# JuliaLinearAlgebra/ArnoldiMethod.jl

Hardware: AMD Instinct MI355X
Metric: arnoldi_iters_per_sec (higher is better)
Workload: dtype f64

## Files before the change

arnoldimethod.jl_amd/_lib.py:

```python
from __future__ import annotations

import ctypes as C
import os

_HERE = os.path.dirname(os.path.abspath(__file__))
LIB_PATH = os.path.join(_HERE, "libkschur_hip.so")

KS_OK, KS_ERR_ARGUMENT, KS_ERR_DIMENSION, KS_ERR_HIP, KS_ERR_RCCL, KS_ERR_QR, KS_ERR_INTERNAL, KS_ERR_NO_DEVICE, KS_ERR_OPERATOR, KS_ERR_COMM = range(10)
KS_F64, KS_C64 = 0, 1
KS_I32, KS_I64 = 0, 1
KS_CSR, KS_CSC = 0, 1
LAYOUTS = {-1: "none", 0: "csr", 1: "csr-vi", 2: "csr-dvi", 3: "sell", 4: "sell-vi", 5: "stencil", 6: "csr-cb"}
PLAN_FACTS = ("ptr64", "ni", "nblk", "nlong", "row_gather", "nslices", "sell_entries", "ncolblocks", "cb_rpt", "cb_ni", "nstencil",
              "nstencil_local", "stencil_mask_bytes", "ndvi", "dvi_unroll")
WHICH = {"LM": 0, "LR": 1, "SR": 2, "LI": 3, "SI": 4}


class ArgumentError(ValueError):
    """Julia's ArgumentError (src/run.jl:111-116,123-124,165-174,185; src/ArnoldiMethod.jl:62-63,87-90)."""


class DimensionMismatch(ValueError):
    """Julia's DimensionMismatch (checksquare, src/run.jl:110)."""

# ... 86 lines not shown
    "ks_workspace_fused_rotations": [vp, P(C.c_int), P(C.c_int), P(C.c_int)],
    "ks_workspace_split_rotations": [vp, P(C.c_int)],
    "ks_workspace_deflated_blocks": [vp, P(C.c_int), P(C.c_int)],
    "ks_sstep_partition": [C.c_int, C.c_int, C.c_int, C.c_int, P(C.c_int), C.c_int, P(C.c_int)],
    "ks_workspace_assert_arnoldi": [vp, i32],
    "ks_workspace_provenance": [vp, P(C.c_int)],
    "ks_workspace_check_guard": [vp, P(C.c_int)],
    "ks_workspace_destroy": [vp],
    "ks_workspace_dims": [vp, P(i64), P(C.c_int), P(C.c_int), P(i64)],
    "ks_workspace_H": [vp, P(vp), P(C.c_int)],
    "ks_workspace_Q": [vp, P(vp), P(C.c_int)],
    "ks_workspace_col_ptr": [vp, i32, P(vp)],
    "ks_workspace_set_seed": [vp, u64],
    "ks_col_upload": [vp, i32, vp],
    "ks_col_download": [vp, i32, vp],
    "ks_cols_download": [vp, i32, i32, vp, i64],
    "ks_cols_upload": [vp, i32, i32, vp, i64],
    "ks_col_fill_uniform": [vp, i32, u64],
    "ks_col_norm": [vp, i32, P(dbl)],
    "ks_col_div": [vp, i32, dbl],
    "ks_col_copy": [vp, i32, i32],
    "ks_apply": [vp, vp, i32, i32],
    "ks_debug_apply_shifted": [vp, vp, i32, i32, dbl, dbl, dbl, i32],
    "ks_gemv_t": [vp, i32, i32, vp],
    "ks_gemv_n_sub": [vp, i32, i32, vp],
    "ks_rotate": [vp, i32, i32, i32, vp, i32],
    "ks_basis_times": [vp, i32, i32, vp, i32, i32, vp, i64],
    "ks_orthogonalize": [vp, i32, P(C.c_int)],
    "ks_reinitialize": [vp, i32, vp, P(C.c_int)],
    "ks_iterate_arnoldi": [vp, vp, i32, i32, P(ks_expand_stats)],
    "ks_params_default": [i64, P(ks_params)],
    "ks_partialschur": [vp, vp, P(ks_params), vp, vp, P(ks_history)],
    "ks_restart": [vp, P(ks_params), i32, P(C.c_int), P(C.c_int), P(C.c_int), vp, vp, vp],
    "ks_expand_restart": [vp, vp, P(ks_params), i32, i32, P(C.c_int), P(C.c_int), P(C.c_int), vp, vp, vp, P(ks_expand_stats), vp],
    "ks_profile_enable": [vp, i32],
    "ks_profile_reset": [vp],
    "ks_profile_get": [vp, i32, vp, vp, vp],
    "ks_residual_norms": [vp, vp, i32, P(dbl), P(dbl)],
    "ks_arnoldi_relation": [vp, vp, i32, P(dbl), P(dbl)],
    "ks_vectors_create": [vp, i64, i32, i32, P(vp)],
    "ks_vectors_destroy": [vp],
    "ks_vectors_dims": [vp, P(i64), P(C.c_int), P(C.c_int), P(i64)],
    "ks_vectors_upload": [vp, i32, i32, vp, i64],
    "ks_vectors_download": [vp, i32, i32, vp, i64],
    "ks_vectors_col_ptr": [vp, i32, P(vp)],
    "ks_basis_times_device": [vp, i32, i32, vp, i32, i32, vp],
# ... 59 lines not shown
```

arnoldimethod.jl_amd/api.py:

```python
from __future__ import annotations

import ctypes as C
import math
from dataclasses import dataclass

import numpy as np

from . import _lib
from ._lib import ArgumentError, DimensionMismatch, check

EPS = float(np.finfo(np.float64).eps)
DEFAULT_SEED = 20240917


class Target:
    name = "LM"

    def __repr__(self):
        return f"{self.name}()"


class LM(Target):
    name = "LM"

# ... 814 lines not shown
        return self.cols(0, self.maxdim + 1)

    def fill_uniform(self, j: int, seed: int):
        check(_lib.load().ks_col_fill_uniform(self._h, j, seed))

    def norm(self, j: int) -> float:
        out = C.c_double()
        check(_lib.load().ks_col_norm(self._h, j, C.byref(out)))
        return out.value

    def div(self, j: int, s: float):
        check(_lib.load().ks_col_div(self._h, j, s))

    def copy_col(self, dst: int, src: int):
        check(_lib.load().ks_col_copy(self._h, dst, src))

    def apply(self, A: Operator, jsrc: int, jdst: int):
        _check_op(_lib.load().ks_apply(A._h, self._h, jsrc, jdst), A)

    def apply_shifted(self, A: Operator, jsrc: int, jdst: int, theta, sigma: float, cacheable: bool = False):
        theta = complex(theta)
        _check_op(_lib.load().ks_debug_apply_shifted(A._h, self._h, jsrc, jdst, theta.real, theta.imag, float(sigma), int(bool(cacheable))), A)

    def gemv_t(self, j: int, jv: int) -> np.ndarray:
        h = np.empty(j, dtype=self.dtype)
        check(_lib.load().ks_gemv_t(self._h, j, jv, h.ctypes.data))
        return h

    def gemv_n_sub(self, j: int, jv: int, h):
        h = np.ascontiguousarray(np.asarray(h, dtype=self.dtype))
        check(_lib.load().ks_gemv_n_sub(self._h, j, jv, h.ctypes.data))

    def rotate(self, c0: int, Qblock):
        Qb = np.asfortranarray(np.asarray(Qblock, dtype=self.dtype))
        c, r = Qb.shape
        check(_lib.load().ks_rotate(self._h, c0, c, r, Qb.ctypes.data, c))

    def basis_times(self, c: int, Y) -> np.ndarray:
        Y = np.asarray(Y)
        ydt = np.complex128 if (Y.dtype.kind == "c" or self.dtype.kind == "c") else np.float64
        Yf = np.asfortranarray(Y.astype(ydt))
        out = np.empty((self.n, Yf.shape[1]), dtype=ydt, order="F")
        check(_lib.load().ks_basis_times(self._h, c, Yf.shape[1], Yf.ctypes.data, Yf.shape[0], _dtype_code(ydt), out.ctypes.data, self.n))
        return out

    def basis_times_device(self, c: int, Y) -> "DeviceVectors":
# ... 415 lines not shown
```

arnoldimethod.jl_amd/csrc/ks_backend.hpp:

```cpp
#pragma once
template <class T> struct HipBackend : ks::Backend<T> {
  using D = typename DevT<T>::type;
  ks_operator* op;
  ks_workspace* ws;
  HipBackend(ks_operator* o, ks_workspace* w) : op(o), ws(w) {}

  int64_t n_global() const override { return ws->n_global; }

  void iterate_arnoldi(int from, int to, const ks::Mat<T>& H, ks::ExpandStats& stats) override {
    guarded_expand([&] { iterate_arnoldi_impl(from, to, H, stats, nullptr); });
  }

  bool iterate_arnoldi_early(int from, int to, const ks::Mat<T>& H, ks::ExpandStats& stats, const std::function<void()>& early) override {
    const char* e = std::getenv("KS_EARLY_RESTART");
    const bool on = !(e && e[0] == '0');
    bool done = false;
    guarded_expand([&] { done = iterate_arnoldi_impl(from, to, H, stats, on ? &early : nullptr); });
    return done;
  }

  template <class F> void guarded_expand(F&& f) {
    try {
      f();
    } catch (...) {
// ... 270 lines not shown
    if (!(rest > 0.0)) return 0;
    int nd = 0;
    for (int j = 0; j < nl;) {
      const int w = width[j] == 2 ? 2 : 1;
      const double mag = w == 2 ? std::max(std::abs(lam[j]), std::abs(lam[j + 1])) : std::abs(lam[j]);
      const double growth = std::pow(mag / rest, std::max(1, steps - 1));
      if (!(mag > ratio * rest) || !(growth > 1e3) || nd + w > ksd::kDeflMax) break;
      for (int q = 0; q < w; ++q) ex.push_back(lam[j + q]);
      nd += w;
      j += w;
    }
    return nd;
  }

  void spec_enqueue(const ksd::BlkShifts<D>& sh, int k_now, bool from_true) {
    if (!ws->spec_on || !ws->rot_defer_on || !ws->gate_allowed || ws->sstep_eff < 8 || !op->async_capable || ws->ctx->hc.allreduce != nullptr) return;
    if (from_true && (!ws->true_start_on || ws->maxdim + 1 > 40)) return;
    const int ne = std::min(10, ws->maxdim - k_now - (sizeof(D) == 8 ? 1 : 0));
    if (ne < 2) return;
    if (!ensure_zscratch<D>(ws)) return;
    if (from_true && !true_start_enqueue<D>(ws)) return;
    char* zs = static_cast<char*>(ws->zscratch);
    op->shift_store_cacheable = true;
    for (int i = 0; i < ne; ++i) {
      op->in_scale = 1.0;
      const void* src = i == 0 ? (from_true ? static_cast<const void*>(ws->ztrue) : ws->col(ws->maxdim)) : static_cast<const void*>(zs + (size_t)(i - 1) * ws->ld * sizeof(D));
      double tre, tim;
      if constexpr (sizeof(D) == 8) { tre = sh.theta[i]; tim = 0.0; }
      else { tre = sh.theta[i].x; tim = sh.theta[i].y; }
      op->apply_shifted(src, zs + (size_t)i * ws->ld * sizeof(D), tre, tim, sh.sigma[i], ws->ld, ws->st);
    }
    ws->spec_sh.assign(reinterpret_cast<const char*>(&sh), reinterpret_cast<const char*>(&sh) + sizeof(sh));
    ws->spec_ne = ne;
    ws->spec_true = from_true;
    ws->spec_valid = true;
  }

  void relation_probe(int from, const ks::Mat<T>& H) {
    const int c = from - 2, nc = from;
    hipStream_t s_ = ws->ctx->stream;
    D* scratch = static_cast<D*>(ws->col(from));
    op->in_scale = 1.0;
    op->apply(ws->col(c), ws->col(from), nullptr);
    if (!ws->probe_dev) {
      KS_HIP(hipMalloc(&ws->probe_dev, 16 + (size_t)(ws->maxdim + 2) * 16));
      KS_HIP(hipHostMalloc(&ws->probe_host, 16 + (size_t)(ws->maxdim + 2) * 16, hipHostMallocCoherent | hipHostMallocMapped));
    }
    double* out = static_cast<double*>(ws->probe_dev);
    D* coef_d = reinterpret_cast<D*>(static_cast<char*>(ws->probe_dev) + 16);
    D* coef_h = reinterpret_cast<D*>(static_cast<char*>(ws->probe_host) + 16);
    double fro2 = 0.0;
    for (int j = 0; j < from - 1; ++j)
// ... 381 lines not shown
```

arnoldimethod.jl_amd/csrc/ks_block.hpp:

```cpp
#pragma once



inline bool blk_shape_ok(int dtype, int k, int s) { return ks_blk_shape_ok(dtype == KS_F64 ? 0 : 1, k, s); }
inline std::vector<int> blk_partition(int dtype, int k0, int count, int smax) {
  std::vector<int> out;
  int k = k0;
  while (count > 0) {
    int s = std::min(count, smax);
    while (s > 1 && !blk_shape_ok(dtype, k, s)) --s;
    if (!blk_shape_ok(dtype, k, s)) break;
    out.push_back(s);
    k += s;
    count -= s;
  }
  return out;
}

inline std::vector<std::complex<double>> leja_shifts(const std::vector<std::complex<double>>& ritz, int s, bool real) {
  std::vector<std::complex<double>> pts;
  for (auto z : ritz) {
    if (real) z = std::complex<double>(z.real(), 0.0);
    if (!std::isfinite(z.real()) || !std::isfinite(z.imag())) continue;
    bool dup = false;
// ... 102 lines not shown
  auto* bs = static_cast<ksd::BlkScratch<D>*>(ws->bscr);
  int k = from;
  int first = 1;
  for (int s : sizes) {
    const bool fuse = first && ws->rot_fuse;
    const bool split = fuse && ws->rot_split;
    const bool chain_true = fuse && ws->chain_true;
    ws->rot_fuse = false;
    ws->rot_split = false;
    ws->chain_true = false;
    char* zs = nullptr;
    if (fuse) {
      KS_REQUIRE(ws->zscratch != nullptr, KS_ERR_INTERNAL, "fused rotation without scratch columns (the adoption allocates them)");
      zs = static_cast<char*>(ws->zscratch);
    }
    if (split) {
      rotate_device<D>(ws, 0, ws->rot_cin, ws->rot_rr, ws->rot_out0, -1);
      ws->rot_split_count++;
    }
    auto zcol = [&](int i) -> void* { return fuse ? static_cast<void*>(zs + (size_t)i * ws->ld * sizeof(D)) : ws->col(k + i); };
    op->shift_store_cacheable = s >= 10;
    const int adopted = fuse ? ws->spec_adopt : 0;
    ws->spec_adopt = 0;
    for (int i = adopted; i < s; ++i) {
      double tre, tim;
      if constexpr (sizeof(D) == 8) { tre = sh.theta[i]; tim = 0.0; }
      else { tre = sh.theta[i].x; tim = sh.theta[i].y; }
      op->in_scale = 1.0;
      const void* src = i == 0 ? (fuse ? (chain_true ? static_cast<const void*>(ws->ztrue) : ws->col(ws->maxdim)) : ws->col(k - 1)) : zcol(i - 1);
      op->apply_shifted(src, zcol(i), tre, tim, sh.sigma[i], ws->ld, ws->st);
      if (ndefl > 0) {
        ProfScope ps(cx, KSP_AXPY, nb8 * 2.0 * (ndefl + 1) + nb8);
        if (!ws->defl_part) KS_HIP(hipMalloc(&ws->defl_part, (size_t)ksd::kDeflMax * (1024 + 1) * sizeof(D)));
        const int nbd = (int)std::max<int64_t>(1, std::min<int64_t>(std::min(1024, cx->num_cu * 4), (ws->n + kBlock - 1) / kBlock));
        D* zc = static_cast<D*>(zcol(i));
        const D* U = static_cast<const D*>(ws->col(0));
        D* part = static_cast<D*>(ws->defl_part);
        ksd::k_defl_dots<D><<<nbd, kBlock, 0, s_>>>(U, ws->ld, ndefl, zc, ws->n, part);
        if (!cx->distributed()) {
          ksd::k_defl_apply<D><<<nbd, kBlock, 0, s_>>>(U, ws->ld, ndefl, zc, ws->n, part, nbd, bs->cdefl + (size_t)i * ksd::kDeflMax);
        } else {
          D* red = part + (size_t)ksd::kDeflMax * 1024;
          ksd::k_defl_reduce<D><<<1, kBlock, 0, s_>>>(part, nbd, ndefl, red);
          cx->allreduce(reinterpret_cast<double*>(red), ndefl * (int)(sizeof(D) / 8));
          ksd::k_defl_apply<D><<<nbd, kBlock, 0, s_>>>(U, ws->ld, ndefl, zc, ws->n, red, 1, bs->cdefl + (size_t)i * ksd::kDeflMax);
        }
      }
    }
    if (ndefl > 0) ws->defl_blocks++;
    const int ne = k * s + s * (s + 1) / 2;
    int nb1, nb2;
    auto fin = [&](int stage, int nbp) {
// ... 61 lines not shown
```

arnoldimethod.jl_amd/csrc/ks_hip.hip:

```cpp
#include <hip/hip_runtime.h>
#include <rccl/rccl.h>

#include <signal.h>
#include <unistd.h>

#include <algorithm>
#include <chrono>
#include <cmath>
#include <cstdio>
#include <cstdlib>
#include <cstring>
#include <memory>
#include <stdexcept>
#include <string>
#include <thread>
#include <unordered_map>
#include <vector>

#include "../../include/kschur.h"
#include "ks_driver.hpp"
#include "ks_kernels.hpp"
#include "ks_spmv_march.hpp"
#include "ks_block_kernels.hpp"
#include "ks_block_launch.hpp"
// ... 998 lines not shown
    check_col(ws, jsrc);
    check_col(ws, jdst);
    KS_REQUIRE(jsrc != jdst, KS_ERR_ARGUMENT, "source and destination columns must differ");
    KS_REQUIRE(A->n_local == ws->n && A->dtype == ws->dtype, KS_ERR_DIMENSION, "operator / workspace mismatch");
    KS_REQUIRE(ws->dtype != KS_F64 || theta_im == 0.0, KS_ERR_ARGUMENT, "a Float64 product takes a real shift");
    ws->ctx->use();
    prov_drop(ws);
    materialize(ws);
    reset_state(ws);
    A->in_scale = 1.0;
    const bool saved = A->shift_store_cacheable;
    A->shift_store_cacheable = cacheable_store != 0;
    try {
      A->apply_shifted(ws->col(jsrc), ws->col(jdst), theta_re, theta_im, sigma, ws->ld, ws->st);
      KS_HIP(hipStreamSynchronize(ws->ctx->stream));
    } catch (...) {
      A->shift_store_cacheable = saved;
      throw;
    }
    A->shift_store_cacheable = saved;
  });
}

int ks_gemv_t(ks_workspace* ws, int j, int jv, void* h_host) {
  return guarded([&] {
    check_col(ws, jv);
    KS_REQUIRE(j >= 1 && j <= ws->maxdim + 1 && h_host, KS_ERR_ARGUMENT, "bad arguments");
    ws->ctx->use();
    materialize(ws);
    reset_state(ws);
    dispatch_dtype(ws->dtype, [&](auto tag) { gemv_t<typename DevT<decltype(tag)>::type>(ws, j, jv, h_host); });
  });
}

int ks_gemv_n_sub(ks_workspace* ws, int j, int jv, const void* h_host) {
  return guarded([&] {
    check_col(ws, jv);
    KS_REQUIRE(j >= 1 && j <= ws->maxdim + 1 && h_host, KS_ERR_ARGUMENT, "bad arguments");
    KS_REQUIRE(jv >= j, KS_ERR_ARGUMENT, "the updated column must not be one of the projected-out columns");
    ws->ctx->use();
    prov_drop(ws);
    materialize(ws);
    dispatch_dtype(ws->dtype, [&](auto tag) { gemv_n_sub<typename DevT<decltype(tag)>::type>(ws, j, jv, h_host); });
  });
}

// ... 698 lines not shown
```

arnoldimethod.jl_amd/csrc/ks_operators.hpp:

```cpp
#pragma once
struct ks_operator {
  ks_ctx* ctx = nullptr;
  int64_t n_local = 0, nnz = 0;
  int dtype = KS_F64;
  bool async_capable = true;
  double bytes_per_nnz = 0.0;
  double aux_bytes = 0.0;
  int layout = -1;
  double in_scale = 1.0;
  bool shift_store_cacheable = false;
  virtual ~ks_operator() = default;
  virtual void apply(const void* x, void* y, const DevState* st) = 0;
  virtual void apply_shifted(const void* x, void* y, double theta_re, double theta_im, double sigma, int64_t ld, const DevState* st);
};

namespace {

template <class D> struct CsrOp : ks_operator {
  void* rowptr = nullptr;
  bool ptr64 = false;
  int32_t* colidx = nullptr;
  D* val = nullptr;
  void* blkptr = nullptr;
  int32_t* blkrow = nullptr;
  int nblk = 0;
  std::vector<std::unique_ptr<CsrOp<D>>> cblocks;
  std::vector<char> cb_from_ghost;
  int cb_rpt = 0, cb_ni = 0;
  int ni = 7;
  bool row_gather = false;
  int nlong = 0;
  int32_t* blkpart = nullptr;
  D* lpart = nullptr;
  int32_t* lrow = nullptr;
  int32_t* lfirst = nullptr;
  int nstencil = 0;
// ... 138 lines not shown
        case 5: go(std::integral_constant<int, 5>{}, M1{}); break;
        case 6: go(std::integral_constant<int, 6>{}, M1{}); break;
        case 7: go(std::integral_constant<int, 7>{}, M1{}); break;
        default: go(std::integral_constant<int, 8>{}, M1{}); break;
      }
    }
  }
  ksd::ShiftArg<D> shift_arg() const {
    ksd::ShiftArg<D> a;
    a.on = shift_on ? 1 : 0;
    a.theta = shift_theta;
    a.sigma = shift_sigma;
    return a;
  }
  void apply_shifted(const void* xv, void* yv, double tre, double tim, double sigma, int64_t ld, const DevState* st) override {
    const int fuse = env_int("KS_SHIFT_FUSED", 1);
    const bool fused = fuse && n_local > 0 && nlong == 0;
    if (!fused) { ks_operator::apply_shifted(xv, yv, tre, tim, sigma, ld, st); return; }
    shift_on = true;
    if constexpr (sizeof(D) == 8) shift_theta = tre; else shift_theta = D{tre, tim};
    shift_sigma = sigma;
    try { apply(xv, yv, st); } catch (...) { shift_on = false; throw; }
    shift_on = false;
  }
  void apply(const void* xv, void* yv, const DevState* st) override {
    const D* x = static_cast<const D*>(xv);
    D* y = static_cast<D*>(yv);
    hipStream_t s = ctx->stream;
    const typename Halo<D>::Begun begun = halo.begin(x, st, n_local > 0 && cblocks.empty() && ndvi == 0 && nslices == 0);
    const ksd::HaloFused& hf = begun.hf;
    const D* xg = begun.xg;
    if (n_local > 0 && !cblocks.empty()) {
      ProfScope ps(ctx, KSP_SPMV, (double)nnz * bytes_per_nnz + aux_bytes + 2.0 * sizeof(D) * n_local);
      if (cb_rpt) {
        ksd::CbArgs<D> a{};
        a.nb = (int)cblocks.size();
        for (int b = 0; b < a.nb; ++b) {
          a.rowptr[b] = static_cast<const int32_t*>(cblocks[b]->rowptr);
          a.colidx[b] = cblocks[b]->colidx;
          a.val[b] = cblocks[b]->val;
          a.xb[b] = (!cb_from_ghost.empty() && cb_from_ghost[b]) ? xg : nullptr;
        }
        const int nt = (int)((n_local + (int64_t)kBlock * cb_rpt - 1) / ((int64_t)kBlock * cb_rpt));
        auto go = [&](auto ni_tag, auto rpt_tag) {
          constexpr int NI = decltype(ni_tag)::value, RPT = decltype(rpt_tag)::value;
          if constexpr ((size_t)NI * kBlock * sizeof(D) <= (size_t)ksd::kSpmvCapBytes)
// ... 424 lines not shown
```

arnoldimethod.jl_amd/csrc/ks_spmv_march.hpp:

```cpp
#pragma once

#include <algorithm>
#include <type_traits>

#include "ks_kernels.hpp"

namespace ksd {

typedef double f64x2m __attribute__((ext_vector_type(2)));

__device__ __forceinline__ double and_mask(double p, int bm) {
  const uint64_t u = __builtin_bit_cast(uint64_t, p);
  const uint32_t lo = (uint32_t)u & (uint32_t)bm, hi = (uint32_t)(u >> 32) & (uint32_t)bm;
  return __builtin_bit_cast(double, ((uint64_t)hi << 32) | lo);
}

__device__ __forceinline__ int march_tile(int xcd, int slot, int it, int S, int ntiles, int& tend) {
  const int q = ntiles >> 3, r = ntiles & 7;
  const int t0 = xcd < r ? xcd * (q + 1) : r * (q + 1) + (xcd - r) * q;
  tend = t0 + (xcd < r ? q + 1 : q);
  return t0 + slot + it * S;
}

__device__ __forceinline__ void march_ld16(f64x2m& dst, uint32_t voff, const void* sbase) {
  asm volatile("global_load_dwordx4 %0, %1, %2" : "=v"(dst) : "v"(voff), "s"(sbase) : "memory");
}
__device__ __forceinline__ void march_ld_u16(uint32_t& dst, uint32_t voff, const void* sbase) {
  asm volatile("global_load_ushort %0, %1, %2" : "=v"(dst) : "v"(voff), "s"(sbase) : "memory");
// ... 520 lines not shown
  for (;;) {
    const bool h1 = z + 1 < zi1;
    step(z, mA, mB, first, h1);
    first = false;
    if (!h1) break;
    ++z;
    const bool h2 = z + 1 < zi1;
    step(z, mB, mA, false, h2);
    if (!h2) break;
    ++z;
  }
  asm volatile("s_waitcnt vmcnt(0)" ::: "memory");
}

__device__ __forceinline__ void march_wait_vm(int c) {
  switch (c) {
    case 0: asm volatile("s_waitcnt vmcnt(0)" ::: "memory"); break;
    case 1: asm volatile("s_waitcnt vmcnt(1)" ::: "memory"); break;
    case 2: asm volatile("s_waitcnt vmcnt(2)" ::: "memory"); break;
    case 3: asm volatile("s_waitcnt vmcnt(3)" ::: "memory"); break;
    case 4: asm volatile("s_waitcnt vmcnt(4)" ::: "memory"); break;
    case 5: asm volatile("s_waitcnt vmcnt(5)" ::: "memory"); break;
    case 6: asm volatile("s_waitcnt vmcnt(6)" ::: "memory"); break;
    default: asm volatile("s_waitcnt vmcnt(7)" ::: "memory"); break;
  }
}

template <unsigned ODDM, int TILE, int TW>
__global__ void __launch_bounds__(TW)
    k_spmv_stencil_marchg(const uint16_t* __restrict__ mask2, const StencilDict<double> d, const double* __restrict__ x,
                          double* __restrict__ y, int64_t n, int nzr, const DevState* __restrict__ st, int shifted, double theta,
                          double sigma) {
  constexpr int NSLOT = 7, KOWN = 3, KFM = 0, KFP = 6;
  constexpr unsigned NEARM = 0x3eu;
  constexpr int PPL = TILE / (2 * TW), kWinB = (TILE + 512) * 8, kPieces = (TILE + 512) / 128, kWaves = TW / 64;
  constexpr int kRounds = (kPieces + kWaves - 1) / kWaves;
  static_assert(TW == 256 || TW == 512, "four or eight waves");
  static_assert((PPL == 1 || PPL == 2) && PPL * 2 * TW == TILE, "one or two pairs per lane");
  static_assert(3 * kWinB <= 60 * 1024, "three window buffers in at most 60 KiB");
  static_assert(kRounds + 2 * PPL <= 7, "march_wait_vm counts up to 7");
  if (st && st->breakdown >= 0) return;
  __shared__ __attribute__((aligned(16))) unsigned char win[3][kWinB];
  const int64_t P = d.delta[KFP];
  const int nx = d.delta[5], ny = (int)(P / nx);
  const int nz = (int)(n / P), ntp = (int)((P + TILE - 1) / TILE);
  const int xcd = blockIdx.x & 7, slot = blockIdx.x >> 3;
  int cnt;
  const int tj0 = march_tile(xcd, 0, 0, 0, ntp, cnt);
  cnt -= tj0;
  if (cnt <= 0) return;
  const int zr = slot / cnt, tile = tj0 + slot % cnt;
  if (zr >= nzr) return;
  const int za = (int)((int64_t)zr * nz / nzr), zb = (int)((int64_t)(zr + 1) * nz / nzr);
  const int64_t off0 = (int64_t)tile * TILE;
  const int wave = __builtin_amdgcn_readfirstlane(threadIdx.x >> 6);
  const uint32_t lane_w = (threadIdx.x & 63u) * 16u;
  const uint32_t win0 = (uint32_t)(uintptr_t)&win[0][0];
  const bool plain_st = (shifted & 2) != 0;
  const int nw = (kPieces - wave + kWaves - 1) / kWaves;
  uint32_t lane_b[PPL];
  bool lane_in[PPL];
  bool wave_has[PPL];
  int mA[PPL], mB[PPL];
// ... 138 lines not shown
          }
        }
      }
      v[KFM] = prev[j];
      if (i > 0) finish(z - 1, j, v[KOWN], -1);
      double s0 = 0.0, s1 = 0.0;
#pragma unroll
      for (int k = 0; k < KFP; ++k) {
        const double p0 = mul_nc(d.val[k], v[k].x), p1 = mul_nc(d.val[k], v[k].y);
        s0 = add_(s0, and_mask(p0, k == KFM ? fm : __builtin_amdgcn_sbfe(mA[j], k, 1)));
        s1 = add_(s1, and_mask(p1, k == KFM ? fm : __builtin_amdgcn_sbfe(mB[j], k, 1)));
      }
      acc[j].x = s0;
      acc[j].y = s1;
      prev[j] = v[KOWN];
    }
    bc = bc == 2 ? 0 : bc + 1;
  }
#pragma unroll
  for (int j = 0; j < PPL; ++j) finish(zi1 - 1, j, top[j], zi1 < nz ? -1 : 0);
  asm volatile("s_waitcnt vmcnt(0)" ::: "memory");
}

}
```

arnoldimethod.jl_amd/csrc/ks_stencil_geom.hpp:

```cpp
#pragma once

#include <cstddef>
#include <cstdint>

struct StencilGeom {
  bool box = false;
  int64_t nx = 0, ny = 0, nz = 0;
};

inline uint8_t stencil_box_mask(int64_t x, int64_t y, int64_t z, int64_t nx, int64_t ny, int64_t nz) {
  return (uint8_t)((z > 0 ? 0x01u : 0u) | (y > 0 ? 0x02u : 0u) | (x > 0 ? 0x04u : 0u) | 0x08u | (x < nx - 1 ? 0x10u : 0u) |
                   (y < ny - 1 ? 0x20u : 0u) | (z < nz - 1 ? 0x40u : 0u));
}

inline StencilGeom stencil_geometry(const int32_t* delta, int nslot, int64_t n, const uint8_t* mask8, size_t nmask) {
  StencilGeom g;
  if (nslot != 7 || n <= 0 || !delta || !mask8 || nmask != (size_t)n) return g;
  const int64_t nx = delta[5], P = delta[6];
  if (nx < 2 || P <= nx || P % nx != 0 || n % P != 0) return g;
  if (delta[0] != -P || delta[1] != -nx || delta[2] != -1 || delta[3] != 0 || delta[4] != 1) return g;
  const int64_t ny = P / nx, nz = n / P;
  int64_t r = 0;
  for (int64_t z = 0; z < nz; ++z)
    for (int64_t y = 0; y < ny; ++y)
      for (int64_t x = 0; x < nx; ++x, ++r)
        if (mask8[r] != stencil_box_mask(x, y, z, nx, ny, nz)) return g;
  g.box = true;
  g.nx = nx;
  g.ny = ny;
  g.nz = nz;
  return g;
}
```

include/kschur.h:

```cpp
#ifndef KSCHUR_H
#define KSCHUR_H

#include <stddef.h>
#include <stdint.h>

#ifdef __cplusplus
extern "C" {
#endif

#define KS_VERSION_MAJOR 0
#define KS_VERSION_MINOR 1

enum {
  KS_OK = 0,
  KS_ERR_ARGUMENT = 1,
  KS_ERR_DIMENSION = 2,
  KS_ERR_HIP = 3,
  KS_ERR_RCCL = 4,
  KS_ERR_QR = 5,
  KS_ERR_INTERNAL = 6,
  KS_ERR_NO_DEVICE = 7,
  KS_ERR_OPERATOR = 8,
  KS_ERR_COMM = 9
};
// ... 105 lines not shown
int ks_workspace_split_rotations(const ks_workspace* ws, int* count);
int ks_workspace_deflated_blocks(const ks_workspace* ws, int* blocks, int* columns);
int ks_debug_blk_time(ks_workspace* ws, int k, int s, int which, int reps, int dbg, double* ms_per_launch, int* grid);
int ks_workspace_assert_arnoldi(ks_workspace* ws, int k);
int ks_workspace_provenance(const ks_workspace* ws, int* k);
int ks_workspace_check_guard(ks_workspace* ws, int* intact);
int ks_workspace_dims(const ks_workspace* ws, int64_t* n_local, int* maxdim, int* dtype, int64_t* ldv);
int ks_workspace_H(ks_workspace* ws, void** H, int* ldh);
int ks_workspace_Q(ks_workspace* ws, void** Q, int* ldq);
int ks_workspace_col_ptr(ks_workspace* ws, int j, void** dev_ptr);
int ks_workspace_set_seed(ks_workspace* ws, uint64_t seed);

int ks_col_upload(ks_workspace* ws, int j, const void* host);
int ks_col_download(ks_workspace* ws, int j, void* host);
int ks_cols_download(ks_workspace* ws, int j0, int ncols, void* host, int64_t ldhost);
int ks_cols_upload(ks_workspace* ws, int j0, int ncols, const void* host, int64_t ldhost);
int ks_col_fill_uniform(ks_workspace* ws, int j, uint64_t seed);
int ks_col_norm(ks_workspace* ws, int j, double* out);
int ks_col_div(ks_workspace* ws, int j, double s);
int ks_col_copy(ks_workspace* ws, int dst, int src);
int ks_apply(ks_operator* A, ks_workspace* ws, int jsrc, int jdst);
int ks_debug_apply_shifted(ks_operator* A, ks_workspace* ws, int jsrc, int jdst, double theta_re, double theta_im, double sigma,
                           int cacheable_store);
int ks_gemv_t(ks_workspace* ws, int j, int jv, void* h_host);
int ks_gemv_n_sub(ks_workspace* ws, int j, int jv, const void* h_host);
int ks_rotate(ks_workspace* ws, int c0, int c, int r, const void* Q_host, int ldq);
int ks_basis_times(ks_workspace* ws, int c, int r, const void* Y_host, int ldy, int ydtype,
                   void* out_host, int64_t ldout);

int ks_orthogonalize(ks_workspace* ws, int j, int* ok);
int ks_reinitialize(ks_workspace* ws, int j, const void* v1_host, int* ok);
typedef struct ks_expand_stats {
  int32_t steps;
  int32_t reorth;
  int32_t breakdowns;
  int32_t explicit_steps;
} ks_expand_stats;
int ks_iterate_arnoldi(ks_operator* A, ks_workspace* ws, int from, int to, ks_expand_stats* stats);

typedef struct ks_params {
  int32_t nev;
  int32_t which;
  double tol;
  int32_t mindim;
  int32_t maxdim;
  int32_t restarts;
// ... 103 lines not shown
```

Before: 4948.

## Fuse consecutive shifted stencil SpMVs into one z-marching pair kernel

Adds apply_shifted2, which computes two back-to-back shifted operator applications (A - theta1)/sigma1 then (A - theta2)/sigma2. For 7-point box stencils in f64 it does this in a single z-marching kernel that keeps the intermediate planes in LDS, so the second product reads the first one's output without another full pass over memory. The s-step block expansion and the speculative enqueue now pair up consecutive shifts to use it. In exchange the kernel has hand-counted vmcnt waits for gfx942/gfx950, a larger LDS footprint, and it only applies when there is no deflation and the geometry is a non-distributed box stencil.

```diff
diff --git a/arnoldimethod.jl_amd/_lib.py b/arnoldimethod.jl_amd/_lib.py
--- a/arnoldimethod.jl_amd/_lib.py
+++ b/arnoldimethod.jl_amd/_lib.py
@@ -132,6 +132,7 @@
     "ks_col_copy": [vp, i32, i32],
     "ks_apply": [vp, vp, i32, i32],
     "ks_debug_apply_shifted": [vp, vp, i32, i32, dbl, dbl, dbl, i32],
+    "ks_debug_apply_shifted2": [vp, vp, i32, i32, i32, dbl, dbl, dbl, dbl, dbl, dbl, i32],
     "ks_gemv_t": [vp, i32, i32, vp],
     "ks_gemv_n_sub": [vp, i32, i32, vp],
     "ks_rotate": [vp, i32, i32, i32, vp, i32],
diff --git a/arnoldimethod.jl_amd/api.py b/arnoldimethod.jl_amd/api.py
--- a/arnoldimethod.jl_amd/api.py
+++ b/arnoldimethod.jl_amd/api.py
@@ -860,6 +860,11 @@
         theta = complex(theta)
         _check_op(_lib.load().ks_debug_apply_shifted(A._h, self._h, jsrc, jdst, theta.real, theta.imag, float(sigma), int(bool(cacheable))), A)
 
+    def apply_shifted2(self, A: Operator, jsrc: int, jmid: int, jdst: int, theta1, sigma1: float, theta2, sigma2: float, cacheable: bool = False):
+        theta1, theta2 = complex(theta1), complex(theta2)
+        _check_op(_lib.load().ks_debug_apply_shifted2(A._h, self._h, jsrc, jmid, jdst, theta1.real, theta1.imag, float(sigma1), theta2.real,
+                                                      theta2.imag, float(sigma2), int(bool(cacheable))), A)
+
     def gemv_t(self, j: int, jv: int) -> np.ndarray:
         h = np.empty(j, dtype=self.dtype)
         check(_lib.load().ks_gemv_t(self._h, j, jv, h.ctypes.data))
diff --git a/arnoldimethod.jl_amd/csrc/ks_backend.hpp b/arnoldimethod.jl_amd/csrc/ks_backend.hpp
--- a/arnoldimethod.jl_amd/csrc/ks_backend.hpp
+++ b/arnoldimethod.jl_amd/csrc/ks_backend.hpp
@@ -316,12 +316,22 @@
     if (from_true && !true_start_enqueue<D>(ws)) return;
     char* zs = static_cast<char*>(ws->zscratch);
     op->shift_store_cacheable = true;
+    auto theta_of = [&](int i, double& tre, double& tim) {
+      if constexpr (sizeof(D) == 8) { tre = sh.theta[i]; tim = 0.0; }
+      else { tre = sh.theta[i].x; tim = sh.theta[i].y; }
+    };
     for (int i = 0; i < ne; ++i) {
       op->in_scale = 1.0;
       const void* src = i == 0 ? (from_true ? static_cast<const void*>(ws->ztrue) : ws->col(ws->maxdim)) : static_cast<const void*>(zs + (size_t)(i - 1) * ws->ld * sizeof(D));
       double tre, tim;
-      if constexpr (sizeof(D) == 8) { tre = sh.theta[i]; tim = 0.0; }
-      else { tre = sh.theta[i].x; tim = sh.theta[i].y; }
+      theta_of(i, tre, tim);
+      if (i + 1 < ne) {
+        double tre2, tim2;
+        theta_of(i + 1, tre2, tim2);
+        op->apply_shifted2(src, zs + (size_t)i * ws->ld * sizeof(D), zs + (size_t)(i + 1) * ws->ld * sizeof(D), tre, tim, sh.sigma[i], tre2, tim2, sh.sigma[i + 1], ws->ld, ws->st);
+        ++i;
+        continue;
+      }
       op->apply_shifted(src, zs + (size_t)i * ws->ld * sizeof(D), tre, tim, sh.sigma[i], ws->ld, ws->st);
     }
     ws->spec_sh.assign(reinterpret_cast<const char*>(&sh), reinterpret_cast<const char*>(&sh) + sizeof(sh));
diff --git a/arnoldimethod.jl_amd/csrc/ks_block.hpp b/arnoldimethod.jl_amd/csrc/ks_block.hpp
--- a/arnoldimethod.jl_amd/csrc/ks_block.hpp
+++ b/arnoldimethod.jl_amd/csrc/ks_block.hpp
@@ -148,12 +148,22 @@
     op->shift_store_cacheable = s >= 10;
     const int adopted = fuse ? ws->spec_adopt : 0;
     ws->spec_adopt = 0;
+    auto theta_of = [&](int i, double& tre, double& tim) {
+      if constexpr (sizeof(D) == 8) { tre = sh.theta[i]; tim = 0.0; }
+      else { tre = sh.theta[i].x; tim = sh.theta[i].y; }
+    };
     for (int i = adopted; i < s; ++i) {
       double tre, tim;
-      if constexpr (sizeof(D) == 8) { tre = sh.theta[i]; tim = 0.0; }
-      else { tre = sh.theta[i].x; tim = sh.theta[i].y; }
+      theta_of(i, tre, tim);
       op->in_scale = 1.0;
       const void* src = i == 0 ? (fuse ? (chain_true ? static_cast<const void*>(ws->ztrue) : ws->col(ws->maxdim)) : ws->col(k - 1)) : zcol(i - 1);
+      if (ndefl == 0 && i + 1 < s) {
+        double tre2, tim2;
+        theta_of(i + 1, tre2, tim2);
+        op->apply_shifted2(src, zcol(i), zcol(i + 1), tre, tim, sh.sigma[i], tre2, tim2, sh.sigma[i + 1], ws->ld, ws->st);
+        ++i;
+        continue;
+      }
       op->apply_shifted(src, zcol(i), tre, tim, sh.sigma[i], ws->ld, ws->st);
       if (ndefl > 0) {
         ProfScope ps(cx, KSP_AXPY, nb8 * 2.0 * (ndefl + 1) + nb8);
diff --git a/arnoldimethod.jl_amd/csrc/ks_hip.hip b/arnoldimethod.jl_amd/csrc/ks_hip.hip
--- a/arnoldimethod.jl_amd/csrc/ks_hip.hip
+++ b/arnoldimethod.jl_amd/csrc/ks_hip.hip
@@ -1044,6 +1044,34 @@
   });
 }
 
+int ks_debug_apply_shifted2(ks_operator* A, ks_workspace* ws, int jsrc, int jmid, int jdst, double theta1_re, double theta1_im, double sigma1,
+                            double theta2_re, double theta2_im, double sigma2, int cacheable_store) {
+  return guarded([&] {
+    KS_REQUIRE(A, KS_ERR_ARGUMENT, "null operator");
+    check_col(ws, jsrc);
+    check_col(ws, jmid);
+    check_col(ws, jdst);
+    KS_REQUIRE(jsrc != jmid, KS_ERR_ARGUMENT, "source and destination columns must differ");
+    KS_REQUIRE(A->n_local == ws->n && A->dtype == ws->dtype, KS_ERR_DIMENSION, "operator / workspace mismatch");
+    KS_REQUIRE(ws->dtype != KS_F64 || (theta1_im == 0.0 && theta2_im == 0.0), KS_ERR_ARGUMENT, "a Float64 product takes a real shift");
+    ws->ctx->use();
+    prov_drop(ws);
+    materialize(ws);
+    reset_state(ws);
+    A->in_scale = 1.0;
+    const bool saved = A->shift_store_cacheable;
+    A->shift_store_cacheable = cacheable_store != 0;
+    try {
+      A->apply_shifted2(ws->col(jsrc), ws->col(jmid), ws->col(jdst), theta1_re, theta1_im, sigma1, theta2_re, theta2_im, sigma2, ws->ld, ws->st);
+      KS_HIP(hipStreamSynchronize(ws->ctx->stream));
+    } catch (...) {
+      A->shift_store_cacheable = saved;
+      throw;
+    }
+    A->shift_store_cacheable = saved;
+  });
+}
+
 int ks_gemv_t(ks_workspace* ws, int j, int jv, void* h_host) {
   return guarded([&] {
     check_col(ws, jv);
diff --git a/arnoldimethod.jl_amd/csrc/ks_operators.hpp b/arnoldimethod.jl_amd/csrc/ks_operators.hpp
--- a/arnoldimethod.jl_amd/csrc/ks_operators.hpp
+++ b/arnoldimethod.jl_amd/csrc/ks_operators.hpp
@@ -12,6 +12,11 @@
   virtual ~ks_operator() = default;
   virtual void apply(const void* x, void* y, const DevState* st) = 0;
   virtual void apply_shifted(const void* x, void* y, double theta_re, double theta_im, double sigma, int64_t ld, const DevState* st);
+  virtual void apply_shifted2(const void* x, void* mid, void* y, double theta1_re, double theta1_im, double sigma1, double theta2_re,
+                              double theta2_im, double sigma2, int64_t ld, const DevState* st) {
+    apply_shifted(x, mid, theta1_re, theta1_im, sigma1, ld, st);
+    apply_shifted(mid, y, theta2_re, theta2_im, sigma2, ld, st);
+  }
 };
 
 namespace {
@@ -196,6 +201,52 @@
     shift_sigma = sigma;
     try { apply(xv, yv, st); } catch (...) { shift_on = false; throw; }
     shift_on = false;
+  }
+  bool march_geom_form() const {
+    if constexpr (!std::is_same<D, double>::value) return false;
+    else {
+      if (!(n_local >= 2 && cblocks.empty() && nstencil == 7 && halo.plan.nghost == 0 && smask2 && stencil_mask_bytes == 1)) return false;
+      if (!env_int("KS_STENCIL_PAIRS", 1) || !march_on() || !env_int("KS_MARCH_WINDOW", 1) || !env_int("KS_MARCH_Z", 1) || env_int("KS_MARCH_GEOM", 1) == 0) return false;
+      const int64_t Pz = sdict.delta[6];
+      if (!geom.box || sdict.delta[3] != 0 || sdict.delta[0] != -Pz || (Pz & 1) != 0 || Pz < 8 * 8 * 512 || n_local / Pz < 8) return false;
+      for (int k = 1; k <= 5; ++k)
+        if (std::llabs((long long)sdict.delta[k]) > 256) return false;
+      return true;
+    }
+  }
+  void launch_pair(const double* x, double* mid, double* y, double t1, double s1, double t2, double s2, const DevState* st) {
+    ProfScope ps(ctx, KSP_SPMV, 2.0 * ((double)nnz * bytes_per_nnz + aux_bytes + 2.0 * sizeof(D) * n_local));
+    const int sh = 1 | (shift_plain() ? 2 : 0);
+    const int zr_env = env_int("KS_MARCH_ZR", 0);
+    PairGeom g;
+    g.P = sdict.delta[6];
+    g.n = n_local;
+    g.nz = (int)(n_local / g.P);
+    g.tile = env_int("KS_MARCH_PAIR_TILE", 1024) == 2048 ? 2048 : 1024;
+    g.nzr = zr_env > 0 ? std::max(1, std::min(zr_env, g.nz / 4)) : pair_default_zr(g);
+    const bool nx_odd = (sdict.delta[5] & 1) != 0;
+    auto go = [&](auto odd_tag, auto tile_tag) {
+      if constexpr (std::is_same<D, double>::value)
+        ksd::k_spmv_stencil_marchg2<decltype(odd_tag)::value, decltype(tile_tag)::value><<<pair_grid(g), 512, 0, ctx->stream>>>(sdict, x, mid, y, n_local, g.nzr, st, sh, t1, s1, t2, s2);
+    };
+    using T1 = std::integral_constant<int, 1024>;
+    using T2 = std::integral_constant<int, 2048>;
+    using OE = std::integral_constant<unsigned, 0x14u>;
+    using OO = std::integral_constant<unsigned, 0x36u>;
+    if (g.tile == 1024) { if (nx_odd) go(OO{}, T1{}); else go(OE{}, T1{}); }
+    else { if (nx_odd) go(OO{}, T2{}); else go(OE{}, T2{}); }
+    KS_HIP(hipGetLastError());
+  }
+  void apply_shifted2(const void* xv, void* mv, void* yv, double t1re, double t1im, double s1, double t2re, double t2im, double s2, int64_t ld,
+                      const DevState* st) override {
+    if constexpr (std::is_same<D, double>::value) {
+      if (env_int("KS_MARCH_PAIR", 1) != 0 && env_int("KS_SHIFT_FUSED", 1) && nlong == 0 && in_scale == 1.0 && !ctx->distributed() && xv != mv &&
+          xv != yv && mv != yv && march_geom_form()) {
+        launch_pair(static_cast<const double*>(xv), static_cast<double*>(mv), static_cast<double*>(yv), t1re, s1, t2re, s2, st);
+        return;
+      }
+    }
+    ks_operator::apply_shifted2(xv, mv, yv, t1re, t1im, s1, t2re, t2im, s2, ld, st);
   }
   void apply(const void* xv, void* yv, const DevState* st) override {
     const D* x = static_cast<const D*>(xv);
diff --git a/arnoldimethod.jl_amd/csrc/ks_spmv_march.hpp b/arnoldimethod.jl_amd/csrc/ks_spmv_march.hpp
--- a/arnoldimethod.jl_amd/csrc/ks_spmv_march.hpp
+++ b/arnoldimethod.jl_amd/csrc/ks_spmv_march.hpp
@@ -4,6 +4,11 @@
 #include <type_traits>
 
 #include "ks_kernels.hpp"
+#include "ks_stencil_geom.hpp"
+
+#if defined(__HIP_DEVICE_COMPILE__) && __HIP_DEVICE_COMPILE__ && !defined(__gfx950__) && !defined(__gfx942__)
+#error "ks_spmv_march.hpp: the hand-counted vmcnt waits are written for gfx942 / gfx950"
+#endif
 
 namespace ksd {
 
@@ -570,7 +575,11 @@
     case 4: asm volatile("s_waitcnt vmcnt(4)" ::: "memory"); break;
     case 5: asm volatile("s_waitcnt vmcnt(5)" ::: "memory"); break;
     case 6: asm volatile("s_waitcnt vmcnt(6)" ::: "memory"); break;
-    default: asm volatile("s_waitcnt vmcnt(7)" ::: "memory"); break;
+    case 7: asm volatile("s_waitcnt vmcnt(7)" ::: "memory"); break;
+    case 8: asm volatile("s_waitcnt vmcnt(8)" ::: "memory"); break;
+    case 9: asm volatile("s_waitcnt vmcnt(9)" ::: "memory"); break;
+    case 10: asm volatile("s_waitcnt vmcnt(10)" ::: "memory"); break;
+    default: asm volatile("s_waitcnt vmcnt(11)" ::: "memory"); break;
   }
 }
 
@@ -586,7 +595,7 @@
   static_assert(TW == 256 || TW == 512, "four or eight waves");
   static_assert((PPL == 1 || PPL == 2) && PPL * 2 * TW == TILE, "one or two pairs per lane");
   static_assert(3 * kWinB <= 60 * 1024, "three window buffers in at most 60 KiB");
-  static_assert(kRounds + 2 * PPL <= 7, "march_wait_vm counts up to 7");
+  static_assert(kRounds + 2 * PPL <= 11, "march_wait_vm counts up to 11");
   if (st && st->breakdown >= 0) return;
   __shared__ __attribute__((aligned(16))) unsigned char win[3][kWinB];
   const int64_t P = d.delta[KFP];
@@ -771,4 +780,218 @@
   asm volatile("s_waitcnt vmcnt(0)" ::: "memory");
 }
 
-}
+template <unsigned ODDM, int TILE>
+__global__ void __launch_bounds__(512)
+    k_spmv_stencil_marchg2(const StencilDict<double> d, const double* __restrict__ x, double* __restrict__ y1, double* __restrict__ y2,
+                           int64_t n, int nzr, const DevState* __restrict__ st, int shifted, double theta1, double sigma1, double theta2,
+                           double sigma2) {
+  constexpr int NSLOT = 7, KOWN = 3, KFM = 0, KFP = 6, TW = 512, kWaves = TW / 64;
+  constexpr unsigned NEARM = 0x3eu;
+  constexpr int PPL = TILE / (2 * TW), NS = PPL + 1;
+  constexpr int kXB = (TILE + 1024) * 8, kYB = (TILE + 512) * 8, kRounds = (TILE + 1024) / 128 / kWaves;
+  static_assert(TILE == 1024 || TILE == 2048, "one or two pairs of the tile per lane");
+  static_assert(kRounds * kWaves * 128 == TILE + 1024, "every wave copies the same number of window pieces");
+  static_assert(3 * kXB + 2 * kYB <= (TILE == 1024 ? 80 : 160) * 1024, "three x windows and two y1 windows in the LDS of two / one workgroups per CU");
+  static_assert(kRounds + 4 * PPL <= 11, "march_wait_vm counts up to 11");
+  if (st && st->breakdown >= 0) return;
+  __shared__ __attribute__((aligned(16))) unsigned char lds[3 * kXB + 2 * kYB];
+  PairGeom g;
+  g.P = d.delta[KFP];
+  g.n = n;
+  g.nz = (int)(n / g.P);
+  g.tile = TILE;
+  g.nzr = nzr;
+  const PairItem it = pair_item(g, (int)blockIdx.x);
+  if (!it.valid) return;
+  const int64_t P = g.P;
+  const int nx = d.delta[5], ny = (int)(P / nx), nz = g.nz;
+  const int wave = __builtin_amdgcn_readfirstlane(threadIdx.x >> 6);
+  const int lane = (int)(threadIdx.x & 63u);
+  const uint32_t lds0 = (uint32_t)(uintptr_t)&lds[0];
+  unsigned char* const ywin = &lds[0] + 3 * kXB;
+  const bool plain_st = (shifted & 2) != 0;
+  const bool halo_w = wave < 4;
+  int e[NS];
+  uint32_t lane_b[PPL];
+  bool lane_in[PPL];
+  bool wave_has[PPL];
+  int mA[NS], mB[NS];
+  int nst = 0;
+#pragma unroll
+  for (int j = 0; j < NS; ++j) {
+    if (j < PPL) e[j] = 256 + j * 2 * TW + 2 * (int)threadIdx.x;
+    else e[j] = !halo_w ? 0 : (threadIdx.x < 128 ? 2 * (int)threadIdx.x : TILE + 2 * (int)threadIdx.x);
+    const int64_t o = it.off0 - 256 + e[j];
+    if (j < PPL) {
+      lane_b[j < PPL ? j : 0] = (uint32_t)(j * 2 * TW + 2 * (int)threadIdx.x) * 8u;
+      lane_in[j < PPL ? j : 0] = o + 1 < P;
+      wave_has[j < PPL ? j : 0] = it.off0 + (int64_t)j * 2 * TW + 128 * (int64_t)wave + 1 < P;
+      nst += wave_has[j < PPL ? j : 0] ? 1 : 0;
+    }
+    const int oa = (int)o, ob = oa + 1;
+    const int ya = oa / nx, xa = oa - ya * nx, yb = ob / nx, xb = ob - yb * nx;
+    mA[j] = 0x08 | (ya > 0 ? 0x02 : 0) | (xa > 0 ? 0x04 : 0) | (xa < nx - 1 ? 0x10 : 0) | (ya < ny - 1 ? 0x20 : 0);
+    mB[j] = 0x08 | (yb > 0 ? 0x02 : 0) | (xb > 0 ? 0x04 : 0) | (xb < nx - 1 ? 0x10 : 0) | (yb < ny - 1 ? 0x20 : 0);
+  }
+  auto issue_w = [&](int zz, int buf) {
+#pragma unroll
+    for (int i = 0; i < kRounds; ++i) {
+      const int k = wave + i * kWaves;
+      const PairSrc s = pair_piece(g, it, zz, k);
+      const double* bw = x + s.base;
+      uint32_t ldst = lds0 + (uint32_t)buf * (uint32_t)kXB + (uint32_t)k * 1024u;
+      const uint32_t voff = (uint32_t)pair_lane(s, 2 * lane) * 8u;
+      asm volatile("" : "+s"(bw));
+      asm volatile("" : "+s"(ldst));
+      asm volatile("s_nop 4" ::: "memory");
+      march_glds16(voff, bw, ldst);
+    }
+  };
+  auto near_taps = [&](const unsigned char* w, f64x2m* v) {
+#pragma unroll
+    for (int k = 0; k < NSLOT; ++k) {
+      if ((NEARM >> k) & 1u) {
+        const int off = (int)d.delta[k] * 8;
+        if (((ODDM >> k) & 1u) == 0) {
+          v[k] = *reinterpret_cast<const f64x2m*>(w + off);
+        } else {
+          typedef double f64x2u8 __attribute__((ext_vector_type(2), aligned(8)));
+          const f64x2u8 p = *reinterpret_cast<const f64x2u8*>(w + off);
+          v[k].x = p.x;
+          v[k].y = p.y;
+        }
+      }
+    }
+  };
+  f64x2m prevx[NS];
+  f64x2m top[NS];
+  f64x2m accx[NS];
+  f64x2m y1m[PPL], y1c[PPL], y1n[PPL];
+#pragma unroll
+  for (int j = 0; j < NS; ++j) {
+    accx[j].x = 0.0;
+    accx[j].y = 0.0;
+  }
+#pragma unroll
+  for (int j = 0; j < PPL; ++j) y1m[j] = y1c[j] = y1n[j] = accx[0];
+  {
+    const PairSrc sp = pair_own(g, it, it.zprev), stp = pair_own(g, it, it.ztop);
+    const double* bp = x + sp.base;
+    const double* bt = x + stp.base;
+    asm volatile("" : "+s"(bp));
+    asm volatile("" : "+s"(bt));
+    asm volatile("s_nop 4" ::: "memory");
+#pragma unroll
+    for (int j = 0; j < NS; ++j) march_ld16(prevx[j], (uint32_t)pair_lane(sp, e[j]) * 8u, bp);
+#pragma unroll
+    for (int j = 0; j < NS; ++j) march_ld16(top[j], (uint32_t)pair_lane(stp, e[j]) * 8u, bt);
+  }
+  issue_w(it.p0, 0);
+  if (it.p0 + 1 <= it.p1) issue_w(it.p0 + 1, 1);
+  march_wait_vm(it.p0 + 1 <= it.p1 ? 2 * kRounds : kRounds);
+#pragma unroll
+  for (int j = 0; j < NS; ++j) {
+    asm volatile("" : "+v"(prevx[j]));
+    asm volatile("" : "+v"(top[j]));
+  }
+  int sA = 0, sB = 0, wB = it.p0 + 1 <= it.p1 ? kRounds : 0;
+  int bx = 0;
+  for (int p = it.p0; p <= it.p1 + 2; ++p) {
+    const bool haswin = p <= it.p1;
+    const bool fin = p > it.p0 && p - 1 <= it.p1;
+    if (haswin) march_wait_vm(sA + wB + sB);
+    asm volatile("s_waitcnt lgkmcnt(0)\n\ts_barrier" ::: "memory");
+    int wN = 0, sN = 0;
+    if (p + 2 <= it.p1) {
+      issue_w(p + 2, bx == 0 ? 2 : bx - 1);
+      wN = kRounds;
+    }
+    const int fm = p > 0 ? -1 : 0;
+    const int fpm = p - 1 < nz - 1 ? -1 : 0;
+    const bool st1 = fin && p - 1 >= it.za && p - 1 < it.zb;
+    double* by1 = y1 + ((int64_t)(p - 1) * P + it.off0);
+    asm volatile("" : "+s"(by1));
+#pragma unroll
+    for (int j = 0; j < NS; ++j) {
+      if (j < PPL || halo_w) {
+        f64x2m v[NSLOT];
+        if (haswin) near_taps(&lds[0] + bx * kXB + (e[j] + 256) * 8, v);
+        else v[KOWN] = top[j];
+        if (fin) {
+          double s0 = add_(accx[j].x, and_mask(mul_nc(d.val[KFP], v[KOWN].x), fpm));
+          double s1 = add_(accx[j].y, and_mask(mul_nc(d.val[KFP], v[KOWN].y), fpm));
+          s0 = scl(sub_s(s0, mul_(theta1, prevx[j].x)), sigma1);
+          s1 = scl(sub_s(s1, mul_(theta1, prevx[j].y)), sigma1);
+          f64x2m o2;
+          o2.x = s0;
+          o2.y = s1;
+          *reinterpret_cast<f64x2m*>(ywin + ((p - 1) & 1) * kYB + e[j] * 8) = o2;
+          if (j < PPL) {
+            y1n[j < PPL ? j : 0] = o2;
+            if (st1 && wave_has[j < PPL ? j : 0]) {
+              if (lane_in[j < PPL ? j : 0]) march_st16(lane_b[j < PPL ? j : 0], o2, by1, plain_st);
+            }
+          }
+        }
+        if (haswin) {
+          v[KFM] = prevx[j];
+          double s0 = 0.0, s1 = 0.0;
+#pragma unroll
+          for (int k = 0; k < KFP; ++k) {
+            const double pa = mul_nc(d.val[k], v[k].x), pb = mul_nc(d.val[k], v[k].y);
+            s0 = add_(s0, and_mask(pa, k == KFM ? fm : __builtin_amdgcn_sbfe(mA[j], k, 1)));
+            s1 = add_(s1, and_mask(pb, k == KFM ? fm : __builtin_amdgcn_sbfe(mB[j], k, 1)));
+          }
+          accx[j].x = s0;
+          accx[j].y = s1;
+          prevx[j] = v[KOWN];
+        }
+      }
+    }
+    if (st1) sN += nst;
+    const int q = p - 2;
+    if (q >= it.za && q < it.zb) {
+      const int fm2 = q > 0 ? -1 : 0, fp2 = q < nz - 1 ? -1 : 0;
+      double* by2 = y2 + ((int64_t)q * P + it.off0);
+      asm volatile("" : "+s"(by2));
+#pragma unroll
+      for (int j = 0; j < PPL; ++j) {
+        f64x2m v[NSLOT];
+        near_taps(ywin + (q & 1) * kYB + e[j] * 8, v);
+        v[KFM] = y1m[j];
+        double s0 = 0.0, s1 = 0.0;
+#pragma unroll
+        for (int k = 0; k < KFP; ++k) {
+          const double pa = mul_nc(d.val[k], v[k].x), pb = mul_nc(d.val[k], v[k].y);
+          s0 = add_(s0, and_mask(pa, k == KFM ? fm2 : __builtin_amdgcn_sbfe(mA[j], k, 1)));
+          s1 = add_(s1, and_mask(pb, k == KFM ? fm2 : __builtin_amdgcn_sbfe(mB[j], k, 1)));
+        }
+        s0 = add_(s0, and_mask(mul_nc(d.val[KFP], y1n[j].x), fp2));
+        s1 = add_(s1, and_mask(mul_nc(d.val[KFP], y1n[j].y), fp2));
+        s0 = scl(sub_s(s0, mul_(theta2, v[KOWN].x)), sigma2);
+        s1 = scl(sub_s(s1, mul_(theta2, v[KOWN].y)), sigma2);
+        f64x2m o2;
+        o2.x = s0;
+        o2.y = s1;
+        if (wave_has[j]) {
+          if (lane_in[j]) march_st16(lane_b[j], o2, by2, plain_st);
+        }
+      }
+      sN += nst;
+    }
+    if (fin) {
+#pragma unroll
+      for (int j = 0; j < PPL; ++j) {
+        y1m[j] = y1c[j];
+        y1c[j] = y1n[j];
+      }
+    }
+    sA = sB;
+    sB = sN;
+    wB = wN;
+    bx = bx == 2 ? 0 : bx + 1;
+  }
+  asm volatile("s_waitcnt vmcnt(0)" ::: "memory");
+}
+
+}
diff --git a/arnoldimethod.jl_amd/csrc/ks_stencil_geom.hpp b/arnoldimethod.jl_amd/csrc/ks_stencil_geom.hpp
--- a/arnoldimethod.jl_amd/csrc/ks_stencil_geom.hpp
+++ b/arnoldimethod.jl_amd/csrc/ks_stencil_geom.hpp
@@ -31,3 +31,82 @@
   g.nz = nz;
   return g;
 }
+
+#if defined(__HIPCC__) || defined(__CUDACC__)
+#define KS_GEOM_HD __host__ __device__
+#else
+#define KS_GEOM_HD
+#endif
+
+struct PairGeom {
+  int64_t P = 0, n = 0;
+  int nz = 0, tile = 0;
+  int nzr = 1;
+};
+struct PairItem {
+  bool valid = false;
+  int tile = 0, zr = 0;
+  int za = 0, zb = 0;
+  int p0 = 0, p1 = 0;
+  int zprev = 0, ztop = 0;
+  int64_t off0 = 0;
+};
+struct PairSrc {
+  int64_t base = 0;
+  int shift = 0, rem = 0;
+};
+
+KS_GEOM_HD inline int pair_tiles(const PairGeom& g) { return (int)((g.P + g.tile - 1) / g.tile); }
+KS_GEOM_HD inline int pair_grid(const PairGeom& g) { return 8 * ((pair_tiles(g) + 7) / 8) * g.nzr; }
+KS_GEOM_HD inline int pair_pieces(const PairGeom& g) { return (g.tile + 1024) / 128; }
+KS_GEOM_HD inline int pair_default_zr(const PairGeom& g) {
+  const int cmax = (pair_tiles(g) + 7) / 8, slots = 32 * (g.tile <= 1024 ? 2 : 1);
+  int nzr = 3 * slots / (2 * cmax);
+  if (nzr > g.nz / 8) nzr = g.nz / 8;
+  return nzr < 1 ? 1 : nzr;
+}
+
+KS_GEOM_HD inline PairItem pair_item(const PairGeom& g, int wg) {
+  PairItem it;
+  const int ntp = pair_tiles(g), xcd = wg & 7, slot = wg >> 3;
+  const int q = ntp >> 3, r = ntp & 7;
+  const int t0 = xcd < r ? xcd * (q + 1) : r * (q + 1) + (xcd - r) * q, cnt = xcd < r ? q + 1 : q;
+  if (cnt <= 0) return it;
+  it.zr = slot / cnt;
+  it.tile = t0 + slot % cnt;
+  if (it.zr >= g.nzr) return it;
+  it.za = (int)((int64_t)it.zr * g.nz / g.nzr);
+  it.zb = (int)((int64_t)(it.zr + 1) * g.nz / g.nzr);
+  if (it.za >= it.zb) return it;
+  it.p0 = it.za > 0 ? it.za - 1 : 0;
+  it.p1 = it.zb < g.nz ? it.zb : g.nz - 1;
+  it.zprev = it.p0 > 0 ? it.p0 - 1 : it.p0;
+  it.ztop = it.p1 < g.nz - 1 ? it.p1 + 1 : it.p1;
+  it.off0 = (int64_t)it.tile * g.tile;
+  it.valid = true;
+  return it;
+}
+KS_GEOM_HD inline PairSrc pair_piece(const PairGeom& g, const PairItem& it, int p, int k) {
+  const int64_t s = (int64_t)p * g.P + it.off0 - 512 + 128 * (int64_t)k;
+  PairSrc r;
+  if (s < 0 || s >= g.n) {
+    r.base = 0;
+    r.rem = 128;
+  } else {
+    r.base = s;
+    r.rem = g.n - s < 128 ? (int)(g.n - s) : 128;
+  }
+  return r;
+}
+KS_GEOM_HD inline PairSrc pair_own(const PairGeom& g, const PairItem& it, int z) {
+  const int64_t b = (int64_t)z * g.P + it.off0 - 256;
+  PairSrc r;
+  r.base = b < 0 ? 0 : b;
+  r.shift = (int)(r.base - b);
+  r.rem = g.n - r.base < g.tile + 512 ? (int)(g.n - r.base) : g.tile + 512;
+  return r;
+}
+KS_GEOM_HD inline int pair_lane(const PairSrc& s, int e) {
+  const int dd = e - s.shift;
+  return (dd >= 0 && dd + 2 <= s.rem) ? dd : 0;
+}
diff --git a/include/kschur.h b/include/kschur.h
--- a/include/kschur.h
+++ b/include/kschur.h
@@ -151,6 +151,8 @@
 int ks_apply(ks_operator* A, ks_workspace* ws, int jsrc, int jdst);
 int ks_debug_apply_shifted(ks_operator* A, ks_workspace* ws, int jsrc, int jdst, double theta_re, double theta_im, double sigma,
                            int cacheable_store);
+int ks_debug_apply_shifted2(ks_operator* A, ks_workspace* ws, int jsrc, int jmid, int jdst, double theta1_re, double theta1_im,
+                            double sigma1, double theta2_re, double theta2_im, double sigma2, int cacheable_store);
 int ks_gemv_t(ks_workspace* ws, int j, int jv, void* h_host);
 int ks_gemv_n_sub(ks_workspace* ws, int j, int jv, const void* h_host);
 int ks_rotate(ks_workspace* ws, int c0, int c, int r, const void* Q_host, int ldq);
```

New measurement: 5008 (median of 5 runs). 1.01x the previous value.
